# KLab/YAIK

Hardware: AMD Instinct MI355X
Metric: Mpix/s tile encode (alpha reject + 7 gradient passes + 8x8 range quant), 8K RGBA (higher is better)
Workload: dtype u8/int32 (+f32 mode-selection sums)

## Files before the change

### yaik_amd/csrc/yk_encode2.hip

```cpp
#include "yk_common.h"
#include "yk_curves.h"
#include "yk_device.h"
#include <mutex>

__constant__ float c_curve2[6][16] = YK_CURVE_TABLE;

#define LS YK_LSTRIDE
#ifdef YK_TEST_HOOKS
#define YK2_ABLATE(bit) ((P.ablate & (bit)) != 0)
#else
#define YK2_ABLATE(bit) false
#endif

__device__ __forceinline__ int y2_byte(uint32_t w, int ch) { return (w >> (8 * ch)) & 255; }
__device__ __forceinline__ uint32_t y2_absdiff(uint32_t a, uint32_t b) { uint32_t r; asm("v_sad_u32 %0, %1, %2, 0" : "=v"(r) : "v"(a), "v"(b)); return r; }
__device__ __forceinline__ int y2_round6(int v) { return (v & ~3) | (v >> 6); }
__device__ __forceinline__ int y2_round6p(int v) { v = min(v + 1, 255); return (v & ~3) | (v >> 6); }

typedef short y2s2 __attribute__((ext_vector_type(2)));
typedef unsigned short y2u2 __attribute__((ext_vector_type(2)));
__device__ __forceinline__ y2u2 y2_u2(uint32_t w) { return __builtin_bit_cast(y2u2, w); }
__device__ __forceinline__ y2s2 y2_s2(y2u2 v) { return __builtin_bit_cast(y2s2, v); }
__device__ __forceinline__ y2u2 y2_splat(int v) { const unsigned short t = (unsigned short)v; return (y2u2){ t, t }; }
__device__ __forceinline__ y2s2 y2_splats(int v) { const short t = (short)v; return (y2s2){ t, t }; }
// ... 381 lines not shown
    YK2_STAT(kPassId * 10 + 0, 1); YK2_STAT(kPassId * 10 + 8, __popcll(y2_spread<NX, NY>(viable)));
    if (y2_compact_sweep<SX, SY>(pass, viable, cov, evaluated)) return;
    const unsigned long long accept = y2_full_pass<SX, SY, SMOOTH>(pass, viable);
    if (accept == 0ULL) return;
    YK2_STAT(kPassId * 10 + 6, 1);
    y2_accept<SX, SY>(pass, cov, accept);
}

#define YK2_QROWS 258
#define YK2_QR0 32
#define YK2_QNR 224
#define YK2_QBYTES ((size_t)YK2_QNR * YK2_QROWS * 16)
#define YK2_RCPBYTES ((size_t)256 * sizeof(float))
#define YK2_DEFN1 224
#define YK2_DEFBYTES ((size_t)225 * YK2_DEFN1 * 4)
#define YK2_TABBYTES (YK2_QBYTES + YK2_RCPBYTES + YK2_DEFBYTES)
typedef _Float16 y2h2 __attribute__((ext_vector_type(2)));
__device__ __forceinline__ uint32_t y2_f16_bits(int n) { const _Float16 h = (_Float16)(float)n; return (uint32_t)__builtin_bit_cast(unsigned short, h); }
__global__ void yk_qtab_kernel(uint4* tab) {
    __shared__ int K[6][16];
    const int R = YK2_QR0 + (int)blockIdx.x, t = threadIdx.x;
    if (t < 96) { const int m = t >> 4, i = t & 15; K[m][i] = __float2int_rz(__fmul_rn(c_curve2[m][i], (float)R)); }
    __syncthreads();
    if (t < YK2_QROWS) {
        const int o = t - 2;
        uint32_t md[6], idx = 0;
        for (int m = 0; m < 6; m++) {
            const int cnt = m < 3 ? 16 : 8;
            int best = 1 << 30, bi = 0;
            for (int n = 0; n < cnt; n++) { const int d = abs(K[m][n] - o); if (d < best) { best = d; bi = n; } }
            best = min(best, 255);
            md[m] = y2_f16_bits(best);
            idx |= (uint32_t)bi << (4 * m);
        }
        tab[(size_t)blockIdx.x * YK2_QROWS + t] = make_uint4(md[0] | (md[1] << 16), md[2] | (md[3] << 16), md[4] | (md[5] << 16), idx);
    }
}
struct Y2TileDef { int base, BN, dist, R; };
__device__ __forceinline__ Y2TileDef y2_tile_def(const int min_, const int d8) {
    Y2TileDef d;
    d.base = (min_ * 63 + 112) / 224;
    d.BN = (d.base * 224) / 63;
    const int scale = 223 - d.BN;
    const int dnum = (d8 - 32) * 127 + (scale - 1);
    d.dist = (scale < 0) ? -dnum : dnum / scale;
    d.R = (d.dist * scale) / 127 + 32;
    return d;
}
__global__ void yk_deftab_kernel(uint32_t* tab) {
    const int min_ = blockIdx.x, d8 = 32 + (int)threadIdx.x;
    const Y2TileDef d = y2_tile_def(min_, d8);
    const int R = min(max(d.R, YK2_QR0), YK2_QR0 + YK2_QNR - 1);
    const uint32_t rowBase = (uint32_t)((R - YK2_QR0) * YK2_QROWS + 2 - d.BN + 256);
    tab[min_ * YK2_DEFN1 + (int)threadIdx.x] = rowBase | (((((uint32_t)d.dist & 255u) << 7) | ((uint32_t)d.base & 255u)) << 16);
}

__global__ void yk_selftest_qtab_kernel(const uint4* tab, const uint32_t* deftab, int* mismatches) {
    const int mn = blockIdx.x, mx = threadIdx.x;
    if (mx < mn) return;
    const int min_ = min(mn, 224);
    int diff = mx - min_; if (diff < 16) diff = 16;
    const int d8 = max(diff, 32);
    const Y2TileDef d = y2_tile_def(min_, d8);
    const int BN = d.BN, R = d.R;
    int bad = 0;
    if (R < YK2_QR0 || R >= YK2_QR0 + YK2_QNR || mn - BN < -2) { atomicAdd(mismatches, 1); return; }
    {
        const uint32_t e = deftab[min_ * YK2_DEFN1 + (d8 - 32)];
        if ((e & 0xFFFFu) != (uint32_t)((R - YK2_QR0) * YK2_QROWS + 2 - BN + 256)) bad++;
        if ((e >> 16) != ((((uint32_t)d.dist & 255u) << 7) | ((uint32_t)d.base & 255u))) bad++;
    }
    for (int m = 0; m < 6; m++) {
        const int cnt = m < 3 ? 16 : 8;
        int L[16];
        for (int i = 0; i < cnt; i++) {
            L[i] = __float2int_rz(__fadd_rn((float)BN, __fmul_rn(c_curve2[m][i], (float)R)));
            if (L[i] != BN + __float2int_rz(__fmul_rn(c_curve2[m][i], (float)R))) bad++;
        }
        for (int v = mn; v <= mx; v++) {
            int best = 1 << 30, bi = 0;
            for (int n = 0; n < cnt; n++) { const int dd = abs(L[n] - v); if (dd < best) { best = dd; bi = n; } }
            const uint4 row = tab[(size_t)(R - YK2_QR0) * YK2_QROWS + (v - BN + 2)];
            const uint32_t w = m < 2 ? row.x : (m < 4 ? row.y : row.z);
            const uint32_t hb = (m & 1) ? (w >> 16) : (w & 0xFFFFu);
            const int ix = (row.w >> (4 * m)) & 15;
            if (hb != y2_f16_bits(best) || ix != bi) bad++;
        }
    }
    if (bad) atomicAdd(mismatches, bad);
}

#define YK2_RUN 16
template <int K> __device__ __forceinline__ uint32_t y2_writelane_k(uint32_t v, uint32_t old) { asm("v_writelane_b32 %0, %1, %2" : "+v"(old) : "s"(v), "n"(K)); return old; }
__device__ __forceinline__ uint32_t y2_writelane(uint32_t v, int k, uint32_t old) {
    switch (k) {
        case 0: return y2_writelane_k<0>(v, old); case 1: return y2_writelane_k<1>(v, old); case 2: return y2_writelane_k<2>(v, old);
        case 3: return y2_writelane_k<3>(v, old); case 4: return y2_writelane_k<4>(v, old); case 5: return y2_writelane_k<5>(v, old);
        case 11: return y2_writelane_k<11>(v, old); default: return y2_writelane_k<12>(v, old);
    }
}
#ifdef YK2_TIMING
__device__ unsigned long long g_y2_times[65536 * 16];
#define YK2_PROBE(i) do { if ((i) == 0 && lane == 0 && unit < 65536) { g_y2_times[(size_t)unit * 16 + 10] = 0; g_y2_times[(size_t)unit * 16 + 11] = 0; g_y2_times[(size_t)unit * 16 + 12] = y2_t_entry; g_y2_times[(size_t)unit * 16 + 13] = ((unsigned long long)y2_xcc << 32) | y2_hwid; } if (lane == 0 && unit < 65536) { g_y2_times[(size_t)unit * 16 + 2 * (i)] = __builtin_amdgcn_s_memtime(); g_y2_times[(size_t)unit * 16 + 2 * (i) + 1] = __builtin_amdgcn_s_memrealtime(); } } while (0)
extern "C" int yk_debug_wave_times(unsigned long long* out) { return (int)hipMemcpyFromSymbol(out, HIP_SYMBOL(g_y2_times), sizeof(g_y2_times)); }
#else
#define YK2_PROBE(i) do { } while (0)
#endif
#define YK2_LUTW 84
#ifndef YK2_WIN
#define YK2_WIN 16
#endif
#ifndef YK2_PREF
#define YK2_PREF 8
#endif
#ifndef YK2_RVWIN
#define YK2_RVWIN 8
#endif

#define Y2_QUAD_X 0xB1
#define Y2_QUAD_Y 0x4E
template <int CTRL> __device__ __forceinline__ int y2_quad(int v) { return __builtin_amdgcn_update_dpp(v, v, CTRL, 0xF, 0xF, true); }
template <int CTRL> __device__ __forceinline__ float y2_quad(float v) { return __int_as_float(y2_quad<CTRL>(__float_as_int(v))); }
template <int FIRST> __device__ __forceinline__ void y2_quad_sums(float (&t)[6]) {
#define Y2_QX(i) "v_add_f32_dpp %" #i ", %" #i ", %" #i " quad_perm:[1,0,3,2] row_mask:0xf bank_mask:0xf\n\t"
#define Y2_QY(i) "v_add_f32_dpp %" #i ", %" #i ", %" #i " quad_perm:[2,3,0,1] row_mask:0xf bank_mask:0xf\n\t"
    if (FIRST == 0)
        asm volatile("s_nop 1\n\t" Y2_QX(0) Y2_QX(1) Y2_QX(2) Y2_QX(3) Y2_QX(4) Y2_QX(5) Y2_QY(0) Y2_QY(1) Y2_QY(2) Y2_QY(3) Y2_QY(4) Y2_QY(5)
                     : "+v"(t[0]), "+v"(t[1]), "+v"(t[2]), "+v"(t[3]), "+v"(t[4]), "+v"(t[5]));
    else
        asm volatile("s_nop 1\n\t" Y2_QX(0) Y2_QX(1) Y2_QX(2) Y2_QY(0) Y2_QY(1) Y2_QY(2) : "+v"(t[3]), "+v"(t[4]), "+v"(t[5]));
#undef Y2_QX
#undef Y2_QY
}
__device__ __forceinline__ float y2_row16_sum(float x) {
    x = __fadd_rn(x, y2_quad<Y2_QUAD_X>(x));
    x = __fadd_rn(x, y2_quad<Y2_QUAD_Y>(x));
    x = __fadd_rn(x, __int_as_float(__builtin_amdgcn_update_dpp(0, __float_as_int(x), 0x141, 0xF, 0xF, true)));
    x = __fadd_rn(x, __int_as_float(__builtin_amdgcn_update_dpp(0, __float_as_int(x), 0x140, 0xF, 0xF, true)));
    return x;
}
__device__ __forceinline__ uint32_t y2_byte_x4(uint32_t w, int ch) {
    uint32_t r; const uint32_t two = 2u;
    if (ch == 0) asm("v_lshlrev_b32_sdwa %0, %1, %2 dst_sel:DWORD dst_unused:UNUSED_PAD src0_sel:DWORD src1_sel:BYTE_0" : "=v"(r) : "v"(two), "v"(w));
    else if (ch == 1) asm("v_lshlrev_b32_sdwa %0, %1, %2 dst_sel:DWORD dst_unused:UNUSED_PAD src0_sel:DWORD src1_sel:BYTE_1" : "=v"(r) : "v"(two), "v"(w));
    else asm("v_lshlrev_b32_sdwa %0, %1, %2 dst_sel:DWORD dst_unused:UNUSED_PAD src0_sel:DWORD src1_sel:BYTE_2" : "=v"(r) : "v"(two), "v"(w));
    return r;
}
__device__ __forceinline__ void y2_fma_lo(float& acc, uint32_t h, float w) { asm volatile("v_fma_mix_f32 %0, %1, %2, %0 op_sel_hi:[1,0,0]" : "+v"(acc) : "v"(h), "v"(w)); }
__device__ __forceinline__ void y2_fma_hi(float& acc, uint32_t h, float w) { asm volatile("v_fma_mix_f32 %0, %1, %2, %0 op_sel:[1,0,0] op_sel_hi:[1,0,0]" : "+v"(acc) : "v"(h), "v"(w)); }
__device__ __forceinline__ uint32_t y2_pack3(int r, int g, int b) {
    return __builtin_amdgcn_perm((uint32_t)b, __builtin_amdgcn_perm((uint32_t)g, (uint32_t)r, 0x0C0C0400u), 0x0C040100u);
}

template <bool WANT_DST, bool MODE3>
__global__ __launch_bounds__(64, 4) void yk_encode2_kernel(const YkEncodeParams P) {
    constexpr int kStart = MODE3 ? 3 : 0;
    constexpr int kPixWords = 17 * LS, kLutWords = WANT_DST ? 16 * YK2_LUTW : 0;
    __shared__ __attribute__((aligned(16))) uint32_t s_mem[kPixWords > kLutWords ? kPixWords : kLutWords];
    uint32_t* const s_pix = s_mem;
    uint32_t (*const s_lut)[YK2_LUTW] = reinterpret_cast<uint32_t (*)[YK2_LUTW]>(s_mem);
    __shared__ uint32_t s_bm[24];
    __shared__ uint8_t s_list[64];
    __shared__ __attribute__((aligned(16))) float s_curve[WANT_DST ? 6 : 1][16];
    __shared__ __attribute__((aligned(16))) float s_rcp[256];
    __shared__ __attribute__((aligned(16))) uint32_t s_aux[432];
    uint32_t* const s_lat = s_aux;
    float (*const s_chain)[68] = reinterpret_cast<float (*)[68]>(s_aux);
    float* const s_err = reinterpret_cast<float*>(s_aux + 408);
    __shared__ uint32_t s_range[3 * 64];
    __shared__ __attribute__((aligned(16))) uint32_t s_sp[3 * 4 * 8 + 3 * 4 * 16];

    uint32_t* const s_tile = s_aux + 416;
    __shared__ uint32_t s_iwTest[WANT_DST ? 1024 : 1];
    uint32_t* const s_iw = WANT_DST ? s_iwTest : s_mem;
    uint32_t* const s_park = WANT_DST ? s_iwTest : s_sp;
    static_assert(WANT_DST || kPixWords >= 1024, "index words need 4 KB");

    const int lane = threadIdx.x;
    __builtin_amdgcn_s_setprio(3);
#ifdef YK2_TIMING
    const unsigned long long y2_t_entry = __builtin_amdgcn_s_memrealtime();
    const unsigned y2_hwid = __builtin_amdgcn_s_getreg((4 << 0) | (0 << 6) | (31 << 11)), y2_xcc = __builtin_amdgcn_s_getreg((20 << 0) | (0 << 6) | (31 << 11));
#endif
    typedef const __attribute__((address_space(4))) YkEncodeParams* Y2ParamPtr;
    auto strip = [&](const int slot, const int xcd, const int lane, Y2ParamPtr const Pp) {
    const __attribute__((address_space(4))) YkEncodeParams& P = *Pp;
    const int nBf = P.xBB64 * P.yBB64, nB = nBf * P.nFrames;
    const int grp = slot / (YK2_RUN * 4);
    const int unit = (grp * 8 + ((xcd + grp) & 7)) * (YK2_RUN * 4) + (slot - grp * (YK2_RUN * 4));
    int L = unit >> 2; const int wave = unit & 3;
    const bool spare = L >= nB;
    L = spare ? 0 : L;
    const uint32_t frU = yk_udiv((uint32_t)L, P.divNBf.mul, P.divNBf.shift);
    L -= (int)frU * nBf;
    const size_t fr = frU;
    const int32_t* const pl0 = P.plane[0] + fr * P.fs.plane; const int32_t* const pl1 = P.plane[1] + fr * P.fs.plane; const int32_t* const pl2 = P.plane[2] + fr * P.fs.plane;
    const int BY = (int)yk_udiv((uint32_t)L, P.divXBB64.mul, P.divXBB64.shift), BX = L - BY * P.xBB64;
    const int w = P.w, h = P.h;
    const int mt0 = (BY * 4 + wave) * P.mtW + BX * 4;

    YK2_PROBE(0);
    if (lane < 24) s_bm[lane] = 0;
    typedef uint32_t y2_u32x2 __attribute__((ext_vector_type(2)));
    typedef int32_t y2_i32x4 __attribute__((ext_vector_type(4)));
    y2_u32x2 keep8; y2_i32x4 bnd;
    {
        const int g4 = (lane & 15) * 4, r0 = lane >> 4;
        const int gx = BX * 64 + g4;
        const bool inX = gx + 3 < w;
        const int gxc = min(gx, w - 4);
        const int gyS = BY * 64 + wave * 16;
        const int gyB = min(gyS, P.hAvail - 1);
        const size_t rowBase = (size_t)gyB * (size_t)P.strideElems;
        const char* const b0 = reinterpret_cast<const char*>(pl0 + rowBase);
        const char* const b1 = reinterpret_cast<const char*>(pl1 + rowBase);
        const char* const b2 = reinterpret_cast<const char*>(pl2 + rowBase);
        int4 R[4], G[4], B[4];
#pragma unroll
        for (int k = 0; k < 4; k++) {
            const int rel = min(gyS + r0 + 4 * k, P.hAvail - 1) - gyB;
            const uint32_t off = (uint32_t)(rel * P.strideElems + gxc) * 4u;
            R[k] = *reinterpret_cast<const int4*>(b0 + off);
            G[k] = *reinterpret_cast<const int4*>(b1 + off);
            B[k] = *reinterpret_cast<const int4*>(b2 + off);
        }
        int4 Rb, Gb, Bb;
        {
            const int rel = min(gyS + 16, P.hAvail - 1) - gyB;
            const uint32_t off = (uint32_t)(rel * P.strideElems + gxc) * 4u;
            Rb = *reinterpret_cast<const int4*>(b0 + off);
            Gb = *reinterpret_cast<const int4*>(b1 + off);
            Bb = *reinterpret_cast<const int4*>(b2 + off);
        }
        uint32_t hcol;
        const int hr = min(max(lane - 32, 0), 16);
        {
            const int rel = min(gyS + hr, P.hAvail - 1) - gyB;
            const uint32_t off = (uint32_t)(rel * P.strideElems + min(BX * 64 + 64, w - 1)) * 4u;
            hcol = y2_pack3(*reinterpret_cast<const int32_t*>(b0 + off), *reinterpret_cast<const int32_t*>(b1 + off), *reinterpret_cast<const int32_t*>(b2 + off));
        }
        const float4 rc4 = *reinterpret_cast<const float4*>(P.qtab + YK2_QBYTES + (size_t)lane * 16);
        const uint4* const orow = P.outTab + (wave * YK2_OT_ROWS + (lane & (YK2_OT_ROWS - 1))) * 2;
        const uint4 ta = orow[0], tb = orow[1];
        {
            const bool rowIn = BY * 64 + wave * 16 < h;
            const uintptr_t args = reinterpret_cast<uintptr_t>(Pp);
            const uintptr_t kpIn = reinterpret_cast<uintptr_t>(P.keep) + fr * P.fs.keep + (uintptr_t)(mt0 & ~3);
            const uintptr_t bpIn = reinterpret_cast<uintptr_t>(P.bounds) + fr * 64;
            const uintptr_t kp = (P.keep != nullptr && rowIn) ? kpIn : args, bp = P.bounds != nullptr ? bpIn : args;
            asm volatile("s_load_dwordx2 %0, %2, 0x0\n\ts_load_dwordx4 %1, %3, 0x0" : "=&s"(keep8), "=&s"(bnd) : "s"(kp), "s"(bp));
        }

        __builtin_amdgcn_s_setprio(0);
        if (spare) return;
        {
            const uint32_t frT = frU + P.outFrame0;
            const uint32_t o = ta.x + frT * ta.y + (uint32_t)BX * ta.z + (uint32_t)BY * ta.w;
            s_park[lane] = ((uint32_t)BX < tb.x && (uint32_t)BY < tb.y) ? o : YK2_OT_NONE;
            s_park[64 + lane] = tb.z;
        }
        uint4 o[4], ob;
#pragma unroll
        for (int k = 0; k < 4; k++) {
            o[k] = make_uint4(y2_pack3(R[k].x, G[k].x, B[k].x), y2_pack3(R[k].y, G[k].y, B[k].y), y2_pack3(R[k].z, G[k].z, B[k].z), y2_pack3(R[k].w, G[k].w, B[k].w));
            *reinterpret_cast<uint4*>(&s_pix[(r0 + 4 * k) * LS + g4]) = o[k];
        }
        ob = make_uint4(y2_pack3(Rb.x, Gb.x, Bb.x), y2_pack3(Rb.y, Gb.y, Bb.y), y2_pack3(Rb.z, Gb.z, Bb.z), y2_pack3(Rb.w, Gb.w, Bb.w));
        if (lane < 16) *reinterpret_cast<uint4*>(&s_pix[16 * LS + g4]) = ob;
        if (BX * 64 + 64 > w) {
            if (!inX) {
#pragma unroll
                for (int k = 0; k < 4; k++) *reinterpret_cast<uint4*>(&s_pix[(r0 + 4 * k) * LS + g4]) = make_uint4(o[k].w, o[k].w, o[k].w, o[k].w);
                if (lane < 16) *reinterpret_cast<uint4*>(&s_pix[16 * LS + g4]) = make_uint4(ob.w, ob.w, ob.w, ob.w);
            }
        }
        if (lane >= 32 && lane <= 48) s_pix[hr * LS + 64] = hcol;
        *reinterpret_cast<float4*>(&s_rcp[lane * 4]) = rc4;

    }
    asm volatile("s_waitcnt lgkmcnt(0)" : "+s"(keep8), "+s"(bnd));
    __syncthreads();
    YK2_PROBE(1);

    const int q = lane >> 4, cx = y2_cell_x(lane & 15), cy = y2_cell_y(lane & 15);
    const int bxCell = q * 16 + cx * 4, byCell = wave * 16 + cy * 4;
    const int gxCell = BX * 64 + bxCell, gyCell = BY * 64 + byCell;
    const int lcell = (cy * 4) * LS + bxCell;
    const int lat = cy * 17 + q * 4 + cx;
    const bool mtIn = (BX * 64 + q * 16 < w) && (BY * 64 + wave * 16 < h);

    uint32_t pw[16];
#pragma unroll
    for (int r = 0; r < 4; r++) {
        const uint4 t = *reinterpret_cast<const uint4*>(&s_pix[lcell + r * LS]);
        pw[r * 4 + 0] = t.x; pw[r * 4 + 1] = t.y; pw[r * 4 + 2] = t.z; pw[r * 4 + 3] = t.w;
    }

    unsigned long long cov = 0ULL;
    unsigned long long evaluated = 0ULL;
    {
        bool dead = !mtIn;
        {
            const int lim = 4 * P.rejectFactor + 1;
            const y2u2 rb0 = y2_u2(pw[0] & 0x00FF00FFu), rb1 = y2_u2(pw[1] & 0x00FF00FFu), rb2 = y2_u2(pw[2] & 0x00FF00FFu), rb3 = y2_u2(pw[3] & 0x00FF00FFu);
            const y2u2 ga = y2_u2(__builtin_amdgcn_perm(pw[1], pw[0], 0x0C050C01u)), gb = y2_u2(__builtin_amdgcn_perm(pw[2], pw[1], 0x0C050C01u)),
                       gc = y2_u2(__builtin_amdgcn_perm(pw[3], pw[2], 0x0C050C01u));
            const y2u2 l2 = y2_splat(lim);
            const y2u2 u1 = rb0 + rb2 - rb1 - rb1 + l2, u2 = rb1 + rb3 - rb2 - rb2 + l2, ug = ga + gc - gb - gb + l2;
            const y2u2 um = __builtin_elementwise_max(__builtin_elementwise_max(u1, u2), ug);
            dead |= __builtin_bit_cast(uint32_t, __builtin_elementwise_sub_sat(um, y2_splat(2 * lim))) != 0u;
        }
        const unsigned long long deadLanes = __ballot(dead);
        YK2_STAT(75, 1); YK2_STAT(76, ~deadLanes == 0ULL ? 1 : 0); YK2_STAT(77, __popcll(deadLanes));
        const bool stripInside = (BX * 64 + 64 <= w) && (BY * 64 + wave * 16 + 16 <= h);
        if (~deadLanes != 0ULL && !YK2_ABLATE(2)) {
            auto latticePoint = [&](const int idx) {
                const int lr = (idx * 241) >> 12, lc = idx - lr * 17;
                const uint32_t raw = s_pix[(lr * 4) * LS + lc * 4];
                const uint32_t r6 = (raw & 0x00FCFCFCu) | ((raw >> 6) & 0x00030303u);
                const uint32_t z = (raw & 0x007F7F7Fu) + 0x00010101u;
                const uint32_t inc = (z ^ (raw & 0x00808080u)) | (((z & raw & 0x00808080u) >> 7) * 255u);
                const uint32_t p6 = (inc & 0x00FCFCFCu) | ((inc >> 6) & 0x00030303u);
                s_lat[0 * YK2_LATN + idx] = __builtin_amdgcn_perm(r6, raw, 0x0C040C00u);
                s_lat[1 * YK2_LATN + idx] = __builtin_amdgcn_perm(r6, raw, 0x0C050C01u);
                s_lat[2 * YK2_LATN + idx] = __builtin_amdgcn_perm(r6, raw, 0x0C060C02u);
                s_lat[3 * YK2_LATN + idx] = __builtin_amdgcn_perm(p6, p6, 0x0C010C00u);
                s_lat[4 * YK2_LATN + idx] = __builtin_amdgcn_perm(p6, p6, 0x0C020C02u);
            };
            latticePoint(lane);
            if (lane < YK2_LATN - 64) latticePoint(lane + 64);
            __syncthreads();
            y2s2 rg[16], bb[8];
#pragma unroll
            for (int k = 0; k < 16; k++) rg[k] = y2_rg(pw[k]);
#pragma unroll
            for (int k = 0; k < 8; k++) bb[k] = y2_bb(pw[2 * k], pw[2 * k + 1]);
            const Y2Pass S = { s_lat, lat, cx, cy, rg, bb, deadLanes, stripInside, gxCell, gyCell, w, h, P.rejectFactor, s_bm, bxCell, byCell, s_pix, s_list, s_range, lane };
            if (deadLanes == 0ULL) y2_grad_pass<4, 4, true>(S, cov, evaluated);
            else y2_grad_pass<4, 4>(S, cov, evaluated);
            if (~(cov | deadLanes) != 0ULL) {
                y2_grad_pass<4, 3>(S, cov, evaluated);
                y2_grad_pass<3, 4>(S, cov, evaluated);
                y2_grad_pass<3, 3>(S, cov, evaluated);
                y2_grad_pass<3, 2>(S, cov, evaluated);
                y2_grad_pass<2, 3>(S, cov, evaluated);
                y2_grad_pass<2, 2>(S, cov, evaluated);
            }
#pragma unroll
            for (int r = 0; r < 4; r++) {
                const uint4 t = *reinterpret_cast<const uint4*>(&s_pix[lcell + r * LS]);
                pw[r * 4 + 0] = t.x; pw[r * 4 + 1] = t.y; pw[r * 4 + 2] = t.z; pw[r * 4 + 3] = t.w;
            }
        }
    }
    const int mtIdx = mt0 + q;
    __syncthreads();
    YK2_PROBE(2);
    uint8_t* const small = P.small;
    const uint32_t tabOff = s_park[lane], tabSel = s_park[64 + lane];
    const uint32_t tabVal = (s_bm[tabSel & 31u] >> ((tabSel >> 8) & 31u)) & (~0u >> (tabSel >> 16));
    uint32_t off32 = (uint32_t)lane - 8u < 5u ? tabOff : ~0u;
    uint32_t val32 = (uint32_t)lane - 8u < 3u ? tabVal : 0u;
    {
        if ((uint32_t)lane - 1u < 3u) *(small + tabOff) = (uint8_t)tabVal;
        const unsigned long long t = ((cov >> 2) ^ cov) & 0x0C0C0C0C0C0C0C0CULL;
        const unsigned long long covRM = cov ^ t ^ (t << 2);
        uint32_t off16 = ((lane & 15) == 0 && mtIn) ? P.oCov + (frU * (uint32_t)P.fs.coverage + (uint32_t)mtIdx) * 2u : ~0u;
        uint32_t val16 = (uint32_t)((covRM >> (q * 16)) & 0xFFFFULL);
        if ((uint32_t)lane - 4u < 3u) { off16 = tabOff; val16 = tabVal; }
        if (off16 != ~0u) *reinterpret_cast<uint16_t*>(small + off16) = (uint16_t)val16;
        if (P.pixCache != nullptr) {
            const bool cellIn = (gxCell < w) && (gyCell < h);
            if (cellIn && !((cov >> lane) & 1ULL)) {
                const uint32_t strip = (uint32_t)((BY * 4 + wave) * P.xBB64 + BX);
                uint4* dstp = P.pixCache + (size_t)strip * 256 + lane;
#pragma unroll
                for (int r = 0; r < 4; r++) dstp[r * 64] = make_uint4(pw[r * 4 + 0], pw[r * 4 + 1], pw[r * 4 + 2], pw[r * 4 + 3]);
            }
        }
    }
    YK2_PROBE(3);
    int cxB = 0, cyB = 0, cw = w, chh = P.fullH, discard = 1;
    if (P.bounds != nullptr) {
        const int b0 = bnd.x, b1 = bnd.y, b2 = bnd.z, b3 = bnd.w;
        discard = (b0 == 0 && b1 == 0 && b2 == w && b3 == P.fullH) ? 1 : 0;
        cxB = (b0 >> 3) << 3; cyB = (b1 >> 3) << 3;
        cw = (((b2 + 7) >> 3) << 3) - cxB; chh = (((b3 + 7) >> 3) << 3) - cyB;
    }
    const int cxl = cx & 1, cyl = cy & 1;
    const int tgx = gxCell - cxl * 4, tgyl = gyCell - cyl * 4, tgy = tgyl + P.y0;
    const bool tileIn = (tgx + 8 <= w) && (tgyl + 8 <= h);
    const bool part = tileIn && tgx >= cxB && tgx < cxB + cw && tgy >= cyB && tgy < cyB + chh && (tgx + 8 <= cw) && (tgy + 8 <= chh);
    const uint32_t keep4 = (uint32_t)((((unsigned long long)keep8.y << 32) | keep8.x) >> (8 * (mt0 & 3)));
    const bool keepMT = (P.keep == nullptr) || discard || (mtIn && ((keep4 >> (8 * q)) & 0xFFu) != 0u);
    const bool tileLive = part && keepMT;
    const int l00 = lane & ~3;
    const uint32_t quadN = (uint32_t)((~cov) >> l00) & 15u;
    const int v00 = (int)(quadN & 1u), v01 = (int)((quadN >> 2) & 1u);
    const bool valid = tileLive && ((quadN >> (lane & 3)) & 1u);
    const int nTop = __popc(quadN & 3u), nBot = __popc(quadN >> 2);
    const int tileIdx = (tgyl >> 3) * P.tilesW + (tgx >> 3);
    const size_t T8 = (size_t)P.tilesW * P.tilesH;
    const int tw = lane >> 2;
    const bool writer = ((lane & 3) == 0) && tileIn;
    const unsigned long long validMask = __ballot(valid);
    const bool fullTiles = !WANT_DST && __ballot(tileLive && quadN != 15u && quadN != 0u) == 0ULL;

    {
        const int n16 = (tileLive && !YK2_ABLATE(1)) ? (nTop + nBot) : 0;
        if ((P.tilesW & 7) == 0) {
            if (validMask != 0ULL) {
#pragma unroll
                for (int r = 0; r < 2; r++) {
                    const bool mine = writer && ((cy >> 1) == r);
                    const unsigned long long b0 = __ballot(mine && (n16 & 1)), b1 = __ballot(mine && (n16 & 2)), b2 = __ballot(mine && (n16 & 4));
                    const unsigned long long bd = __ballot(mine && n16 > 0);
                    val32 = y2_writelane((uint32_t)(__popcll(b0) + 2 * __popcll(b1) + 4 * __popcll(b2)) | ((uint32_t)__popcll(bd) << 16), 11 + r, val32);
                }
            }
        } else if (writer && n16 > 0) {
            uint32_t* const blockCntP = P.blockCnt + fr * P.fs.blockN;
            atomicAdd(&blockCntP[((size_t)tileIdx >> 10) * 2], 16u * (uint32_t)n16);
            atomicAdd(&blockCntP[((size_t)tileIdx >> 10) * 2 + 1], 1u);
        }
        if (off32 != ~0u) *reinterpret_cast<uint32_t*>(small + off32) = val32;
    }

    YK2_STAT(70, validMask != 0ULL ? 1 : 0); YK2_STAT(74, __popcll(validMask));
    { const int nv = __popcll(validMask); YK2_STAT(120 + (nv == 0 ? 0 : nv <= 4 ? 1 : nv <= 8 ? 2 : nv <= 16 ? 3 : nv <= 32 ? 4 : nv < 64 ? 5 : 6), 1); (void)nv; }
    uint32_t defs01 = 0u, defs2c = 0u;
    if (validMask != 0ULL && !YK2_ABLATE(1)) {
        uint8_t* const slotsP = P.slots + fr * P.fs.slots;
        uint32_t* lut = &s_lut[WANT_DST ? tw : 0][0];
        if (WANT_DST) {
            s_curve[lane >> 4][lane & 15] = c_curve2[lane >> 4][lane & 15];
            if (lane < 32) s_curve[4 + (lane >> 4)][lane & 15] = c_curve2[4 + (lane >> 4)][lane & 15];
        }
        const int j4 = lane & 3;
        const int nValidLanes = __popcll(validMask);
        const bool spread = nValidLanes <= 4 && !WANT_DST;
        const int vRank = (int)__builtin_amdgcn_mbcnt_hi((uint32_t)(validMask >> 32), __builtin_amdgcn_mbcnt_lo((uint32_t)validMask, 0u));
        uint32_t slotOff[4];
#pragma unroll
        for (int r = 0; r < 4; r++) {
            const int yIn = cyl * 4 + r;
            const int pos = (yIn < 4) ? (yIn * 4 * nTop + (cxl ? 4 * v00 : 0))
                                      : (16 * nTop + (yIn - 4) * 4 * nBot + (cxl ? 4 * v01 : 0));
            slotOff[r] = (uint32_t)tileIdx * (uint32_t)YK_SLOT + (uint32_t)(pos >> 1);
        }
        int tmn[3], tmx[3];
        {
            y2u2 mnRB = y2_splat(0xFFFF), mxRB = y2_splat(0), mnG = y2_splat(0xFFFF), mxG = y2_splat(0);
            if (valid) {
#pragma unroll
                for (int k = 0; k < 16; k += 2) {
                    const y2u2 a = y2_u2(pw[k] & 0x00FF00FFu), b = y2_u2(pw[k + 1] & 0x00FF00FFu), g = y2_u2(__builtin_amdgcn_perm(pw[k + 1], pw[k], 0x0C050C01u));
                    if (k == 0) { mnRB = __builtin_elementwise_min(a, b); mxRB = __builtin_elementwise_max(a, b); mnG = g; mxG = g; }
                    else {
                        mnRB = __builtin_elementwise_min(__builtin_elementwise_min(mnRB, a), b); mxRB = __builtin_elementwise_max(__builtin_elementwise_max(mxRB, a), b);
                        mnG = __builtin_elementwise_min(mnG, g); mxG = __builtin_elementwise_max(mxG, g);
                    }
                }
            }
            tmn[0] = (int)mnRB.x; tmn[2] = (int)mnRB.y; tmx[0] = (int)mxRB.x; tmx[2] = (int)mxRB.y;
            tmn[1] = min((int)mnG.x, (int)mnG.y); tmx[1] = max((int)mxG.x, (int)mxG.y);
#pragma unroll
            for (int p = 0; p < 3; p++) {
                tmn[p] = min(tmn[p], y2_quad<Y2_QUAD_X>(tmn[p])); tmx[p] = max(tmx[p], y2_quad<Y2_QUAD_X>(tmx[p]));
                tmn[p] = min(tmn[p], y2_quad<Y2_QUAD_Y>(tmn[p])); tmx[p] = max(tmx[p], y2_quad<Y2_QUAD_Y>(tmx[p]));
            }
        }
        const uint32_t* const defTab = reinterpret_cast<const uint32_t*>(P.qtab + YK2_QBYTES + YK2_RCPBYTES);
        uint32_t tdef[3];
#pragma unroll
        for (int p = 0; p < 3; p++) {
            const int none = tmn[p] > 255;
            const int mn = none ? 0 : tmn[p], mx = none ? 0 : tmx[p];
            const int min_ = min(mn, 224);
            const int d8 = max(mx - min_, 32);
            tdef[p] = defTab[(uint32_t)(min_ * YK2_DEFN1 + d8 - 32)];
            s_range[p * 64 + lane] = (uint32_t)mn | ((uint32_t)mx << 8);
        }
        const uint8_t* const qrows = P.qtab - (size_t)256 * 16;
        if (spread && !YK2_ABLATE(4)) {
            if (valid) s_list[vRank] = (uint8_t)lane;
            __builtin_amdgcn_fence(__ATOMIC_RELEASE, "wavefront"); __builtin_amdgcn_wave_barrier(); __builtin_amdgcn_fence(__ATOMIC_ACQUIRE, "wavefront");
            const int spI = lane >> 4, spK = lane & 15;
            const bool spAct = spI < nValidLanes;
            const int spSrc = (int)s_list[spAct ? spI : 0];
            const int sq = spSrc >> 4, scx = y2_cell_x(spSrc & 15), scy = y2_cell_y(spSrc & 15);
            const uint32_t spx = s_pix[(scy * 4 + (spK >> 2)) * LS + sq * 16 + scx * 4 + (spK & 3)];
#pragma unroll
            for (int p = 0; p < 3; p++) {
                const uint32_t q16s = (uint32_t)__builtin_amdgcn_ds_bpermute(spSrc << 2, (int)((tdef[p] & 0xFFFFu) << 4));
                float t6[6] = { 0.0f, 0.0f, 0.0f, 0.0f, 0.0f, 0.0f };
                if (spAct) {
                    const uint32_t v4 = y2_byte_x4(spx, p);
                    const uint4 row = *reinterpret_cast<const uint4*>(qrows + (size_t)((v4 << 2) + q16s));
                    const float rv = *reinterpret_cast<const float*>(reinterpret_cast<const char*>(s_rcp) + v4);
                    if (!MODE3) { y2_fma_lo(t6[0], row.x, rv); y2_fma_hi(t6[1], row.x, rv); y2_fma_lo(t6[2], row.y, rv); }
                    y2_fma_hi(t6[3], row.y, rv); y2_fma_lo(t6[4], row.z, rv); y2_fma_hi(t6[5], row.z, rv);
                    s_sp[96 + (p * 4 + spI) * 16 + spK] = row.w;
                }
#pragma unroll
                for (int m = kStart; m < 6; m++) {
                    const float tot = y2_row16_sum(t6[m]);
                    if (spK == 0) s_sp[(p * 4 + spI) * 8 + m] = __float_as_uint(tot);
                }
            }
            __builtin_amdgcn_fence(__ATOMIC_RELEASE, "wavefront"); __builtin_amdgcn_wave_barrier(); __builtin_amdgcn_fence(__ATOMIC_ACQUIRE, "wavefront");
        }
        uint4 win[16];
        auto issueRows = [&](const int pl, const int k0, const int k1) {
            if (valid && !spread && !YK2_ABLATE(4)) {
                const uint32_t q16 = (tdef[pl] & 0xFFFFu) << 4;
                {
#pragma unroll
                    for (int k = k0; k < k1; k++) {
                        const uint32_t v4 = y2_byte_x4(pw[k], pl);
                        win[k] = *reinterpret_cast<const uint4*>(qrows + (size_t)((v4 << 2) + q16));
                    }
                }
            }
        };
        issueRows(0, 0, YK2_PREF);
#pragma unroll
        for (int p = 0; p < 3; p++) {
            const uint32_t qrow16 = (tdef[p] & 0xFFFFu) << 4;
            float sm[6] = { 0.0f, 0.0f, 0.0f, 0.0f, 0.0f, 0.0f };
            issueRows(p, YK2_PREF, 16);
            if (valid && !spread && !YK2_ABLATE(4)) {
                float rvw[YK2_RVWIN];
                auto issueRcp = [&](const int k, float& rv) { rv = *reinterpret_cast<const float*>(reinterpret_cast<const char*>(s_rcp) + y2_byte_x4(pw[k], p)); };
#pragma unroll
                for (int k = 0; k < YK2_RVWIN; k++) issueRcp(k, rvw[k]);
#pragma unroll
                for (int k = 0; k < 16; k++) {
                    __builtin_amdgcn_sched_barrier(0);
                    const uint4 row = win[k]; const float rv = rvw[k % YK2_RVWIN];
                    if (!MODE3) { y2_fma_lo(sm[0], row.x, rv); y2_fma_hi(sm[1], row.x, rv); y2_fma_lo(sm[2], row.y, rv); }
                    y2_fma_hi(sm[3], row.y, rv); y2_fma_lo(sm[4], row.z, rv); y2_fma_hi(sm[5], row.z, rv);
                    s_iw[k * 64 + lane] = row.w;
                    if (k + YK2_RVWIN < 16) issueRcp(k + YK2_RVWIN, rvw[k % YK2_RVWIN]);
                }
                __builtin_amdgcn_sched_barrier(0);
            }
            if (spread && valid && !YK2_ABLATE(4)) {
#pragma unroll
                for (int m = kStart; m < 6; m++) sm[m] = __uint_as_float(s_sp[(p * 4 + vRank) * 8 + m]);
#pragma unroll
                for (int k4 = 0; k4 < 4; k4++) {
                    const uint4 iw4 = *reinterpret_cast<const uint4*>(&s_sp[96 + (p * 4 + vRank) * 16 + k4 * 4]);
                    s_iw[(k4 * 4 + 0) * 64 + lane] = iw4.x; s_iw[(k4 * 4 + 1) * 64 + lane] = iw4.y; s_iw[(k4 * 4 + 2) * 64 + lane] = iw4.z; s_iw[(k4 * 4 + 3) * 64 + lane] = iw4.w;
                }
            }
            if (p < 2) issueRows(p + 1, 0, YK2_PREF);
            float tm[6] = { sm[0], sm[1], sm[2], sm[3], sm[4], sm[5] };
            y2_quad_sums<kStart>(tm);
            int bestMode = kStart; float bestT = tm[kStart];
            bool near = false;
#pragma unroll
            for (int m = kStart + 1; m < 6; m++) {
                const float t = tm[m];
                const float lo = fminf(t, bestT), hi = fmaxf(t, bestT);
                near |= !(__fmul_rn(lo, 1.00002f) < hi);
                bestMode = (t <= bestT) ? m : bestMode;
                bestT = lo;
            }
            bool amb = false;
            uint32_t ties = 0;
            if (__ballot(near && tileLive) != 0ULL) {
                int bm = kStart; float bt = tm[kStart];
#pragma unroll
                for (int m = kStart + 1; m < 6; m++) {
                    const float t = tm[m];
                    const float lo = fminf(t, bt), hi = fmaxf(t, bt);
                    const bool eq = (t == bt);
                    amb |= !eq && !(__fmul_rn(lo, 1.00002f) < hi);
                    if (eq && t != 0.0f) ties |= (1u << m) | ((uint32_t)bm << (8 + 3 * m));
                    bm = (t <= bt) ? m : bm;
                    bt = lo;
                }
            }
            if (__ballot(ties != 0u && tileLive) != 0ULL) {
// ... 75 lines not shown
#pragma unroll
                for (int m = 3; m < 6; m++) {
                    uint32_t Lq[2];
#pragma unroll
                    for (int k = 0; k < 2; k++)
                        Lq[k] = (uint32_t)__float2int_rz(__fadd_rn(BNf, __fmul_rn(s_curve[m][j4 * 2 + k], Rf)));
                    *reinterpret_cast<uint2*>(&lut[60 + (m - 3) * 8 + j4 * 2]) = make_uint2(Lq[0] << 8, Lq[1] << 8);
                }
                __builtin_amdgcn_fence(__ATOMIC_RELEASE, "wavefront");
                __builtin_amdgcn_wave_barrier();
                __builtin_amdgcn_fence(__ATOMIC_ACQUIRE, "wavefront");
            }
            while (ambMask != 0ULL) {
                const int a00 = (__ffsll((long long)ambMask) - 1) & ~3;
                ambMask &= ~(0xFULL << a00);
                if (l00 == a00) {
#pragma unroll
                    for (int r = 0; r < 4; r++) {
                        const uint32_t kSel = 0x0C0C0000u | ((4u + (uint32_t)p) << 8) | (uint32_t)p;
                        const uint32_t lo2 = __builtin_amdgcn_perm(pw[r * 4 + 1], pw[r * 4 + 0], kSel), hi2 = __builtin_amdgcn_perm(pw[r * 4 + 3], pw[r * 4 + 2], kSel);
                        s_tile[(cyl * 4 + r) * 2 + cxl] = __builtin_amdgcn_perm(hi2, lo2, 0x05040100u);
                    }
                }
                const uint32_t tq16 = (uint32_t)__builtin_amdgcn_readlane((int)qrow16, a00), tqn = (uint32_t)__builtin_amdgcn_readlane((int)quadN, a00);
                __builtin_amdgcn_fence(__ATOMIC_RELEASE, "wavefront");
                __builtin_amdgcn_wave_barrier();
                __builtin_amdgcn_fence(__ATOMIC_ACQUIRE, "wavefront");
                {
                    const uint32_t v = (uint32_t)reinterpret_cast<const uint8_t*>(s_tile)[lane];
                    const bool pv = ((tqn >> (((lane >> 5) << 1) | ((lane >> 2) & 1))) & 1u) != 0u;
                    uint4 rw = make_uint4(0u, 0u, 0u, 0u);
                    if (pv) rw = *reinterpret_cast<const uint4*>(qrows + (size_t)((v << 4) + tq16));
                    const float fv = (float)v, rr = pv ? s_rcp[v] : 0.0f;
                    const y2h2 h01 = __builtin_bit_cast(y2h2, rw.x), h23 = __builtin_bit_cast(y2h2, rw.y), h45 = __builtin_bit_cast(y2h2, rw.z);
                    s_chain[0][lane] = yk_div_exact((float)h01.x, fv, rr);
                    s_chain[1][lane] = yk_div_exact((float)h01.y, fv, rr);
                    s_chain[2][lane] = yk_div_exact((float)h23.x, fv, rr);
                    s_chain[3][lane] = yk_div_exact((float)h23.y, fv, rr);
                    s_chain[4][lane] = yk_div_exact((float)h45.x, fv, rr);
                    s_chain[5][lane] = yk_div_exact((float)h45.y, fv, rr);
                }
                __builtin_amdgcn_fence(__ATOMIC_RELEASE, "wavefront");
                __builtin_amdgcn_wave_barrier();
                __builtin_amdgcn_fence(__ATOMIC_ACQUIRE, "wavefront");
                if (lane < 6 && lane >= kStart) {
                    float sacc = 0.0f;
                    const float4* cp = reinterpret_cast<const float4*>(&s_chain[lane][0]);
#pragma unroll
                    for (int k = 0; k < 16; k++) {
                        const float4 a = cp[k];
                        sacc = __fadd_rn(__fadd_rn(__fadd_rn(__fadd_rn(sacc, a.x), a.y), a.z), a.w);
                    }
                    s_err[lane] = sacc;
                }
                __builtin_amdgcn_fence(__ATOMIC_RELEASE, "wavefront");
                __builtin_amdgcn_wave_barrier();
                __builtin_amdgcn_fence(__ATOMIC_ACQUIRE, "wavefront");
                if (l00 == a00) {
                    bestMode = -1; float bestErr = 99999999.0f;
                    for (int m = kStart; m < 6; m++) {
                        const float e = s_err[m];
                        if (e <= bestErr) { bestErr = e; bestMode = m; }
                    }
                    if (valid) {
                        const uint32_t sh = 4u * (uint32_t)bestMode;
#pragma unroll
                        for (int k = 0; k < 16; k++) {
                            const uint32_t code = s_iw[k * 64 + lane] >> sh;
                            if (k < 8) cLo = __builtin_amdgcn_alignbit(code, cLo, 4); else cHi = __builtin_amdgcn_alignbit(code, cHi, 4);
                        }
                    }
                }
                __builtin_amdgcn_wave_barrier();
            }
            if (valid && fullTiles) {
                uint8_t* const slotPlane = slotsP + (size_t)p * T8 * YK_SLOT;
                const uint32_t nLo = (uint32_t)y2_quad<Y2_QUAD_X>((int)cLo), nHi = (uint32_t)y2_quad<Y2_QUAD_X>((int)cHi);
                if (cxl == 0) {
                    uint32_t so = slotOff[0];
                    asm volatile("" : "+v"(so));
                    const uint4 half = make_uint4(__builtin_amdgcn_perm(nLo, cLo, 0x05040100u), __builtin_amdgcn_perm(nLo, cLo, 0x07060302u),
                                                  __builtin_amdgcn_perm(nHi, cHi, 0x05040100u), __builtin_amdgcn_perm(nHi, cHi, 0x07060302u));
                    *reinterpret_cast<uint4*>(slotPlane + so) = half;
                }
            } else if (valid) {
                uint8_t* const slotPlane = slotsP + (size_t)p * T8 * YK_SLOT;
#pragma unroll
                for (int r = 0; r < 4; r++) {
                    const uint32_t code16 = ((r < 2 ? cLo : cHi) >> (16 * (r & 1))) & 0xFFFFu;
                    uint32_t so = slotOff[r];
                    asm volatile("" : "+v"(so));
                    *reinterpret_cast<uint16_t*>(slotPlane + so) = (uint16_t)code16;
                    if (WANT_DST) {
                        const uint32_t* lb = lut + (bestMode < 3 ? bestMode * 20 : 60 + (bestMode - 3) * 8);
                        int32_t* drow = P.dst[p] + (uint32_t)((gyCell + r) * w + gxCell);
#pragma unroll
                        for (int i = 0; i < 4; i++) drow[i] = (int32_t)(lb[(code16 >> (4 * i)) & 15u] >> 8);
                    }
                }
            }
            {
                const uint32_t def16 = (((uint32_t)bestMode & 255u) << 13) | (tdef[p] >> 16);
                if (p == 0) defs01 = def16 & 0xFFFFu; else if (p == 1) defs01 |= def16 << 16; else defs2c = def16 & 0xFFFFu;
            }
            __builtin_amdgcn_wave_barrier();
        }
        defs2c |= (uint32_t)(tileLive ? 16 * (nTop + nBot) : 0) << 16;
    }
    if (writer) {
        const uint32_t offI = P.oInfo + (frU * (uint32_t)P.fs.tileInfo + (uint32_t)tileIdx) * 8u;
        *reinterpret_cast<uint2*>(small + offI) = make_uint2(defs01, defs2c);
    }
    YK2_PROBE(4);
    };
    strip((int)blockIdx.x >> 3, (int)blockIdx.x & 7, lane, (Y2ParamPtr)__builtin_amdgcn_kernarg_segment_ptr());
}

static uint8_t* g_qtab[64] = {};
static std::mutex g_qtabMu;
int yk_qtab_get(yk_ctx* c) {
    std::lock_guard<std::mutex> guard(g_qtabMu);
    if (c->device < 0 || c->device >= 64) return yk_fail(c, YK_ERR_BAD_ARG, "device index");
    if (!g_qtab[c->device]) {
        uint8_t* t = nullptr;
        YK_HIP(c, hipMalloc(&t, 4096 + YK2_TABBYTES));
        YK_HIP(c, hipMemsetAsync(t, 0, 4096, c->stream));
        t += 4096;
        hipLaunchKernelGGL(yk_qtab_kernel, dim3(YK2_QNR), dim3(320), 0, c->stream, reinterpret_cast<uint4*>(t));
        {
            float rcp[256]; rcp[0] = 0.0f;
            for (int v = 1; v < 256; v++) rcp[v] = 1.0f / (float)v;
            YK_HIP(c, hipMemcpyAsync(t + YK2_QBYTES, rcp, sizeof rcp, hipMemcpyHostToDevice, c->stream));
        }
        hipLaunchKernelGGL(yk_deftab_kernel, dim3(225), dim3(YK2_DEFN1), 0, c->stream, reinterpret_cast<uint32_t*>(t + YK2_QBYTES + YK2_RCPBYTES));
        YK_HIP(c, hipGetLastError());
        YK_HIP(c, hipStreamSynchronize(c->stream));
        g_qtab[c->device] = t;
    }
    c->qtab = g_qtab[c->device];
    return YK_OK;
}
void yk_selftest_qtab_launch(yk_ctx* c, int* mismatches) {
    hipLaunchKernelGGL(yk_selftest_qtab_kernel, dim3(256), dim3(256), 0, c->stream, reinterpret_cast<const uint4*>(c->qtab),
                       reinterpret_cast<const uint32_t*>(c->qtab + YK2_QBYTES + YK2_RCPBYTES), mismatches);
}

int yk_launch_encode2(yk_ctx* c, const YkEncodeParams& P) {
    if (!P.qtab) return yk_fail(c, YK_ERR_STATE, "quantiser table missing");
    if (P.startMode != 0 && P.startMode != 3) return yk_fail(c, YK_ERR_BAD_ARG, "startMode must be 0 or 3");
    const int nB = P.xBB64 * P.yBB64 * P.nFrames, group = 8 * YK2_RUN;
    if ((long long)P.xBB64 * P.yBB64 * P.nFrames + group > (long long)YK_UDIV_LIMIT) return yk_fail(c, YK_ERR_BAD_ARG, "too many blocks for one launch");
    if (!P.outTab) return yk_fail(c, YK_ERR_STATE, "output table missing");
    dim3 grid(((nB + group - 1) / group) * group * 4);
    if (P.wantDst) {
        if (P.startMode) hipLaunchKernelGGL((yk_encode2_kernel<true, true>), grid, dim3(64), 0, c->stream, P);
        else hipLaunchKernelGGL((yk_encode2_kernel<true, false>), grid, dim3(64), 0, c->stream, P);
    } else {
        if (P.startMode) hipLaunchKernelGGL((yk_encode2_kernel<false, true>), grid, dim3(64), 0, c->stream, P);
        else hipLaunchKernelGGL((yk_encode2_kernel<false, false>), grid, dim3(64), 0, c->stream, P);
    }
    YK_HIP(c, hipGetLastError());
    return YK_OK;
}
```

Baseline: 240,900.

## Add whole-image aligned specialization of encode kernel skipping edge clamps

Adds a WHOLE template variant that runs when the image is single-frame, 64-aligned and needs no sub-window or destination output. It drops the frame division, the row and column clamps and the edge padding, and computes the tile-live mask per strip with one box test instead of per-lane checks. It also defers reloading pixel words from shared memory until after the valid-mask check, so strips with no valid tiles skip that reload. The cost is an extra kernel instantiation and separate code paths whose correctness depends on the host-side eligibility check.

```diff
diff --git a/yaik_amd/csrc/yk_encode2.hip b/yaik_amd/csrc/yk_encode2.hip
--- a/yaik_amd/csrc/yk_encode2.hip
+++ b/yaik_amd/csrc/yk_encode2.hip
@@ -557,7 +557,7 @@
     return __builtin_amdgcn_perm((uint32_t)b, __builtin_amdgcn_perm((uint32_t)g, (uint32_t)r, 0x0C0C0400u), 0x0C040100u);
 }
 
-template <bool WANT_DST, bool MODE3>
+template <bool WANT_DST, bool MODE3, bool WHOLE = false>
 __global__ __launch_bounds__(64, 4) void yk_encode2_kernel(const YkEncodeParams P) {
     constexpr int kStart = MODE3 ? 3 : 0;
     constexpr int kPixWords = 17 * LS, kLutWords = WANT_DST ? 16 * YK2_LUTW : 0;
@@ -590,13 +590,13 @@
     typedef const __attribute__((address_space(4))) YkEncodeParams* Y2ParamPtr;
     auto strip = [&](const int slot, const int xcd, const int lane, Y2ParamPtr const Pp) {
     const __attribute__((address_space(4))) YkEncodeParams& P = *Pp;
-    const int nBf = P.xBB64 * P.yBB64, nB = nBf * P.nFrames;
+    const int nBf = P.xBB64 * P.yBB64, nB = WHOLE ? nBf : nBf * P.nFrames;
     const int grp = slot / (YK2_RUN * 4);
     const int unit = (grp * 8 + ((xcd + grp) & 7)) * (YK2_RUN * 4) + (slot - grp * (YK2_RUN * 4));
     int L = unit >> 2; const int wave = unit & 3;
     const bool spare = L >= nB;
     L = spare ? 0 : L;
-    const uint32_t frU = yk_udiv((uint32_t)L, P.divNBf.mul, P.divNBf.shift);
+    const uint32_t frU = WHOLE ? 0u : yk_udiv((uint32_t)L, P.divNBf.mul, P.divNBf.shift);
     L -= (int)frU * nBf;
     const size_t fr = frU;
     const int32_t* const pl0 = P.plane[0] + fr * P.fs.plane; const int32_t* const pl1 = P.plane[1] + fr * P.fs.plane; const int32_t* const pl2 = P.plane[2] + fr * P.fs.plane;
@@ -612,15 +612,45 @@
     {
         const int g4 = (lane & 15) * 4, r0 = lane >> 4;
         const int gx = BX * 64 + g4;
-        const bool inX = gx + 3 < w;
-        const int gxc = min(gx, w - 4);
+        const bool inX = WHOLE || gx + 3 < w;
+        const int gxc = WHOLE ? gx : min(gx, w - 4);
         const int gyS = BY * 64 + wave * 16;
+        int4 R[4], G[4], B[4], Rb, Gb, Bb;
+        uint32_t hcol;
+        int hr;
+        if constexpr (WHOLE) {
+            const int stride = P.strideElems;
+            const size_t base = (size_t)gyS * (size_t)stride + (size_t)(BX * 64);
+            const char* const b0 = reinterpret_cast<const char*>(pl0 + base);
+            const char* const b1 = reinterpret_cast<const char*>(pl1 + base);
+            const char* const b2 = reinterpret_cast<const char*>(pl2 + base);
+            const uint32_t offL = (uint32_t)(r0 * stride + g4) * 4u;
+#pragma unroll
+            for (int k = 0; k < 4; k++) {
+                const uint32_t off = offL + (uint32_t)(k * 16 * stride);
+                R[k] = *reinterpret_cast<const int4*>(b0 + off);
+                G[k] = *reinterpret_cast<const int4*>(b1 + off);
+                B[k] = *reinterpret_cast<const int4*>(b2 + off);
+            }
+            const int relB = min(gyS + 16, h - 1) - gyS;
+            {
+                const uint32_t off = (uint32_t)(relB * stride) * 4u + (uint32_t)g4 * 4u;
+                Rb = *reinterpret_cast<const int4*>(b0 + off);
+                Gb = *reinterpret_cast<const int4*>(b1 + off);
+                Bb = *reinterpret_cast<const int4*>(b2 + off);
+            }
+            hr = min(max(lane - 32, 0), 16);
+            {
+                const int colH = min(BX * 64 + 64, w - 1) - BX * 64;
+                const uint32_t off = (uint32_t)(min(hr, relB) * stride + colH) * 4u;
+                hcol = y2_pack3(*reinterpret_cast<const int32_t*>(b0 + off), *reinterpret_cast<const int32_t*>(b1 + off), *reinterpret_cast<const int32_t*>(b2 + off));
+            }
+        } else {
         const int gyB = min(gyS, P.hAvail - 1);
         const size_t rowBase = (size_t)gyB * (size_t)P.strideElems;
         const char* const b0 = reinterpret_cast<const char*>(pl0 + rowBase);
         const char* const b1 = reinterpret_cast<const char*>(pl1 + rowBase);
         const char* const b2 = reinterpret_cast<const char*>(pl2 + rowBase);
-        int4 R[4], G[4], B[4];
 #pragma unroll
         for (int k = 0; k < 4; k++) {
             const int rel = min(gyS + r0 + 4 * k, P.hAvail - 1) - gyB;
@@ -629,7 +659,6 @@
             G[k] = *reinterpret_cast<const int4*>(b1 + off);
             B[k] = *reinterpret_cast<const int4*>(b2 + off);
         }
-        int4 Rb, Gb, Bb;
         {
             const int rel = min(gyS + 16, P.hAvail - 1) - gyB;
             const uint32_t off = (uint32_t)(rel * P.strideElems + gxc) * 4u;
@@ -637,18 +666,18 @@
             Gb = *reinterpret_cast<const int4*>(b1 + off);
             Bb = *reinterpret_cast<const int4*>(b2 + off);
         }
-        uint32_t hcol;
-        const int hr = min(max(lane - 32, 0), 16);
+        hr = min(max(lane - 32, 0), 16);
         {
             const int rel = min(gyS + hr, P.hAvail - 1) - gyB;
             const uint32_t off = (uint32_t)(rel * P.strideElems + min(BX * 64 + 64, w - 1)) * 4u;
             hcol = y2_pack3(*reinterpret_cast<const int32_t*>(b0 + off), *reinterpret_cast<const int32_t*>(b1 + off), *reinterpret_cast<const int32_t*>(b2 + off));
         }
+        }
         const float4 rc4 = *reinterpret_cast<const float4*>(P.qtab + YK2_QBYTES + (size_t)lane * 16);
         const uint4* const orow = P.outTab + (wave * YK2_OT_ROWS + (lane & (YK2_OT_ROWS - 1))) * 2;
         const uint4 ta = orow[0], tb = orow[1];
         {
-            const bool rowIn = BY * 64 + wave * 16 < h;
+            const bool rowIn = WHOLE || BY * 64 + wave * 16 < h;
             const uintptr_t args = reinterpret_cast<uintptr_t>(Pp);
             const uintptr_t kpIn = reinterpret_cast<uintptr_t>(P.keep) + fr * P.fs.keep + (uintptr_t)(mt0 & ~3);
             const uintptr_t bpIn = reinterpret_cast<uintptr_t>(P.bounds) + fr * 64;
@@ -661,7 +690,7 @@
         {
             const uint32_t frT = frU + P.outFrame0;
             const uint32_t o = ta.x + frT * ta.y + (uint32_t)BX * ta.z + (uint32_t)BY * ta.w;
-            s_park[lane] = ((uint32_t)BX < tb.x && (uint32_t)BY < tb.y) ? o : YK2_OT_NONE;
+            s_park[lane] = (WHOLE || ((uint32_t)BX < tb.x && (uint32_t)BY < tb.y)) ? o : YK2_OT_NONE;
             s_park[64 + lane] = tb.z;
         }
         uint4 o[4], ob;
@@ -672,7 +701,7 @@
         }
         ob = make_uint4(y2_pack3(Rb.x, Gb.x, Bb.x), y2_pack3(Rb.y, Gb.y, Bb.y), y2_pack3(Rb.z, Gb.z, Bb.z), y2_pack3(Rb.w, Gb.w, Bb.w));
         if (lane < 16) *reinterpret_cast<uint4*>(&s_pix[16 * LS + g4]) = ob;
-        if (BX * 64 + 64 > w) {
+        if (!WHOLE && BX * 64 + 64 > w) {
             if (!inX) {
 #pragma unroll
                 for (int k = 0; k < 4; k++) *reinterpret_cast<uint4*>(&s_pix[(r0 + 4 * k) * LS + g4]) = make_uint4(o[k].w, o[k].w, o[k].w, o[k].w);
@@ -692,7 +721,7 @@
     const int gxCell = BX * 64 + bxCell, gyCell = BY * 64 + byCell;
     const int lcell = (cy * 4) * LS + bxCell;
     const int lat = cy * 17 + q * 4 + cx;
-    const bool mtIn = (BX * 64 + q * 16 < w) && (BY * 64 + wave * 16 < h);
+    const bool mtIn = WHOLE || ((BX * 64 + q * 16 < w) && (BY * 64 + wave * 16 < h));
 
     uint32_t pw[16];
 #pragma unroll
@@ -700,6 +729,7 @@
         const uint4 t = *reinterpret_cast<const uint4*>(&s_pix[lcell + r * LS]);
         pw[r * 4 + 0] = t.x; pw[r * 4 + 1] = t.y; pw[r * 4 + 2] = t.z; pw[r * 4 + 3] = t.w;
     }
+    bool ranPasses = false;
 
     unsigned long long cov = 0ULL;
     unsigned long long evaluated = 0ULL;
@@ -717,7 +747,7 @@
         }
         const unsigned long long deadLanes = __ballot(dead);
         YK2_STAT(75, 1); YK2_STAT(76, ~deadLanes == 0ULL ? 1 : 0); YK2_STAT(77, __popcll(deadLanes));
-        const bool stripInside = (BX * 64 + 64 <= w) && (BY * 64 + wave * 16 + 16 <= h);
+        const bool stripInside = WHOLE || ((BX * 64 + 64 <= w) && (BY * 64 + wave * 16 + 16 <= h));
         if (~deadLanes != 0ULL && !YK2_ABLATE(2)) {
             auto latticePoint = [&](const int idx) {
                 const int lr = (idx * 241) >> 12, lc = idx - lr * 17;
@@ -751,10 +781,13 @@
                 y2_grad_pass<2, 3>(S, cov, evaluated);
                 y2_grad_pass<2, 2>(S, cov, evaluated);
             }
-#pragma unroll
-            for (int r = 0; r < 4; r++) {
-                const uint4 t = *reinterpret_cast<const uint4*>(&s_pix[lcell + r * LS]);
-                pw[r * 4 + 0] = t.x; pw[r * 4 + 1] = t.y; pw[r * 4 + 2] = t.z; pw[r * 4 + 3] = t.w;
+            if constexpr (WHOLE) ranPasses = true;
+            else {
+#pragma unroll
+                for (int r = 0; r < 4; r++) {
+                    const uint4 t = *reinterpret_cast<const uint4*>(&s_pix[lcell + r * LS]);
+                    pw[r * 4 + 0] = t.x; pw[r * 4 + 1] = t.y; pw[r * 4 + 2] = t.z; pw[r * 4 + 3] = t.w;
+                }
             }
         }
     }
@@ -775,45 +808,70 @@
         if ((uint32_t)lane - 4u < 3u) { off16 = tabOff; val16 = tabVal; }
         if (off16 != ~0u) *reinterpret_cast<uint16_t*>(small + off16) = (uint16_t)val16;
         if (P.pixCache != nullptr) {
-            const bool cellIn = (gxCell < w) && (gyCell < h);
+            const bool cellIn = WHOLE || ((gxCell < w) && (gyCell < h));
             if (cellIn && !((cov >> lane) & 1ULL)) {
                 const uint32_t strip = (uint32_t)((BY * 4 + wave) * P.xBB64 + BX);
                 uint4* dstp = P.pixCache + (size_t)strip * 256 + lane;
 #pragma unroll
-                for (int r = 0; r < 4; r++) dstp[r * 64] = make_uint4(pw[r * 4 + 0], pw[r * 4 + 1], pw[r * 4 + 2], pw[r * 4 + 3]);
+                for (int r = 0; r < 4; r++)
+                    dstp[r * 64] = WHOLE ? *reinterpret_cast<const uint4*>(&s_pix[lcell + r * LS]) : make_uint4(pw[r * 4 + 0], pw[r * 4 + 1], pw[r * 4 + 2], pw[r * 4 + 3]);
             }
         }
     }
     YK2_PROBE(3);
-    int cxB = 0, cyB = 0, cw = w, chh = P.fullH, discard = 1;
+    int cxB = 0, cyB = 0, cw = w, chh = WHOLE ? h : P.fullH, discard = 1;
     if (P.bounds != nullptr) {
         const int b0 = bnd.x, b1 = bnd.y, b2 = bnd.z, b3 = bnd.w;
-        discard = (b0 == 0 && b1 == 0 && b2 == w && b3 == P.fullH) ? 1 : 0;
+        discard = (b0 == 0 && b1 == 0 && b2 == w && b3 == (WHOLE ? h : P.fullH)) ? 1 : 0;
         cxB = (b0 >> 3) << 3; cyB = (b1 >> 3) << 3;
         cw = (((b2 + 7) >> 3) << 3) - cxB; chh = (((b3 + 7) >> 3) << 3) - cyB;
     }
     const int cxl = cx & 1, cyl = cy & 1;
-    const int tgx = gxCell - cxl * 4, tgyl = gyCell - cyl * 4, tgy = tgyl + P.y0;
-    const bool tileIn = (tgx + 8 <= w) && (tgyl + 8 <= h);
-    const bool part = tileIn && tgx >= cxB && tgx < cxB + cw && tgy >= cyB && tgy < cyB + chh && (tgx + 8 <= cw) && (tgy + 8 <= chh);
-    const uint32_t keep4 = (uint32_t)((((unsigned long long)keep8.y << 32) | keep8.x) >> (8 * (mt0 & 3)));
-    const bool keepMT = (P.keep == nullptr) || discard || (mtIn && ((keep4 >> (8 * q)) & 0xFFu) != 0u);
-    const bool tileLive = part && keepMT;
+    const int tgx = gxCell - cxl * 4, tgyl = gyCell - cyl * 4, tgy = WHOLE ? tgyl : tgyl + P.y0;
+    const bool tileIn = WHOLE || ((tgx + 8 <= w) && (tgyl + 8 <= h));
+    bool tileLive, valid;
+    unsigned long long validMask, liveMask = 0ULL;
+    bool askLanes = false;
+    if constexpr (WHOLE) {
+        const int sx0 = BX * 64, sy0 = BY * 64 + wave * 16;
+        const bool inBox = sx0 >= cxB && sx0 + 56 < cxB + cw && sy0 >= cyB && sy0 + 8 < cyB + chh && (sx0 + 64 <= cw) && (sy0 + 16 <= chh);
+        askLanes = !inBox;
+        if (inBox) {
+            const uint32_t k4 = keep8.x;
+            liveMask = ~0ULL;
+            if (P.keep != nullptr && !discard)
+                liveMask = ((k4 & 0x000000FFu) ? 0x000000000000FFFFULL : 0ULL) | ((k4 & 0x0000FF00u) ? 0x00000000FFFF0000ULL : 0ULL) |
+                           ((k4 & 0x00FF0000u) ? 0x0000FFFF00000000ULL : 0ULL) | ((k4 & 0xFF000000u) ? 0xFFFF000000000000ULL : 0ULL);
+        }
+    }
+    if (!WHOLE || askLanes) {
+        const bool part = tileIn && tgx >= cxB && tgx < cxB + cw && tgy >= cyB && tgy < cyB + chh && (tgx + 8 <= cw) && (tgy + 8 <= chh);
+        const uint32_t keep4 = (uint32_t)((((unsigned long long)keep8.y << 32) | keep8.x) >> (8 * (mt0 & 3)));
+        const bool keepMT = (P.keep == nullptr) || discard || (mtIn && ((keep4 >> (8 * q)) & 0xFFu) != 0u);
+        tileLive = part && keepMT;
+        if constexpr (WHOLE) liveMask = __ballot(tileLive);
+    }
+    if constexpr (WHOLE) {
+        validMask = liveMask & ~cov;
+        tileLive = __builtin_amdgcn_inverse_ballot_w64(liveMask);
+        valid = __builtin_amdgcn_inverse_ballot_w64(validMask);
+    }
     const int l00 = lane & ~3;
     const uint32_t quadN = (uint32_t)((~cov) >> l00) & 15u;
     const int v00 = (int)(quadN & 1u), v01 = (int)((quadN >> 2) & 1u);
-    const bool valid = tileLive && ((quadN >> (lane & 3)) & 1u);
+    if constexpr (!WHOLE) valid = tileLive && ((quadN >> (lane & 3)) & 1u);
     const int nTop = __popc(quadN & 3u), nBot = __popc(quadN >> 2);
     const int tileIdx = (tgyl >> 3) * P.tilesW + (tgx >> 3);
     const size_t T8 = (size_t)P.tilesW * P.tilesH;
     const int tw = lane >> 2;
     const bool writer = ((lane & 3) == 0) && tileIn;
-    const unsigned long long validMask = __ballot(valid);
-    const bool fullTiles = !WANT_DST && __ballot(tileLive && quadN != 15u && quadN != 0u) == 0ULL;
+    if constexpr (!WHOLE) validMask = __ballot(valid);
+    bool fullTiles = false;
+    if constexpr (!WHOLE) fullTiles = !WANT_DST && __ballot(tileLive && quadN != 15u && quadN != 0u) == 0ULL;
 
     {
         const int n16 = (tileLive && !YK2_ABLATE(1)) ? (nTop + nBot) : 0;
-        if ((P.tilesW & 7) == 0) {
+        if (WHOLE || (P.tilesW & 7) == 0) {
             if (validMask != 0ULL) {
 #pragma unroll
                 for (int r = 0; r < 2; r++) {
@@ -835,6 +893,16 @@
     { const int nv = __popcll(validMask); YK2_STAT(120 + (nv == 0 ? 0 : nv <= 4 ? 1 : nv <= 8 ? 2 : nv <= 16 ? 3 : nv <= 32 ? 4 : nv < 64 ? 5 : 6), 1); (void)nv; }
     uint32_t defs01 = 0u, defs2c = 0u;
     if (validMask != 0ULL && !YK2_ABLATE(1)) {
+        if constexpr (WHOLE) {
+            if (ranPasses) {
+#pragma unroll
+                for (int r = 0; r < 4; r++) {
+                    const uint4 t = *reinterpret_cast<const uint4*>(&s_pix[lcell + r * LS]);
+                    pw[r * 4 + 0] = t.x; pw[r * 4 + 1] = t.y; pw[r * 4 + 2] = t.z; pw[r * 4 + 3] = t.w;
+                }
+            }
+            fullTiles = __ballot(tileLive && quadN != 15u && quadN != 0u) == 0ULL;
+        }
         uint8_t* const slotsP = P.slots + fr * P.fs.slots;
         uint32_t* lut = &s_lut[WANT_DST ? tw : 0][0];
         if (WANT_DST) {
@@ -1216,7 +1284,14 @@
     if ((long long)P.xBB64 * P.yBB64 * P.nFrames + group > (long long)YK_UDIV_LIMIT) return yk_fail(c, YK_ERR_BAD_ARG, "too many blocks for one launch");
     if (!P.outTab) return yk_fail(c, YK_ERR_STATE, "output table missing");
     dim3 grid(((nB + group - 1) / group) * group * 4);
-    if (P.wantDst) {
+    bool whole = !P.wantDst && P.nFrames == 1 && P.y0 == 0 && P.hAvail == P.h && P.fullH == P.h && (P.w & 63) == 0 && (P.h & 63) == 0 && (P.tilesW & 7) == 0;
+#ifdef YK_TEST_HOOKS
+    if (P.ablate & 32) whole = false;
+#endif
+    if (whole) {
+        if (P.startMode) hipLaunchKernelGGL((yk_encode2_kernel<false, true, true>), grid, dim3(64), 0, c->stream, P);
+        else hipLaunchKernelGGL((yk_encode2_kernel<false, false, true>), grid, dim3(64), 0, c->stream, P);
+    } else if (P.wantDst) {
         if (P.startMode) hipLaunchKernelGGL((yk_encode2_kernel<true, true>), grid, dim3(64), 0, c->stream, P);
         else hipLaunchKernelGGL((yk_encode2_kernel<true, false>), grid, dim3(64), 0, c->stream, P);
     } else {
```

Result: faster. 244,900 (median of 6 runs) (+1.7%).
